# tenstack/batch-scheduler

Measured on AMD Instinct MI355X. Metric: pod x node fit evals/sec, higher is better.
Workload: dtype int64; 1 GPU; cfg3/tail: 10000 pods / 2000 groups / 5000 nodes, 5 int64 lanes (cpu, mem, eph, pods, gpu), seed 20260921; stages=prefilter+filter+tally+ready, parallelism=single GPU

## Files before the change

### batch-scheduler_amd/csrc/bs_fast.hpp

```cpp
#pragma once

#include "bs_kernels.hpp"
#include "bs_filter_t.hpp"

#ifdef BS_NT_TABLES
#define BS_TBL_STORE(p, v) __builtin_nontemporal_store((v), (p))
#else
#define BS_TBL_STORE(p, v) (*(p) = (v))
#endif
namespace bs {

template <bool INL = false>
__device__ __forceinline__ void arm_tally(const GroupsDev& gr, const BatchDev& b, const BatchParams& prm, uint32_t i, uint32_t nthreads);

__device__ __forceinline__ const uint8_t* range_glocal(const BatchDev& b) { return reinterpret_cast<const uint8_t*>(b.pod_ranges); }
__device__ __forceinline__ const uint32_t* range_start(const BatchDev& b, uint32_t G) { return b.pod_ranges + (G + 3u) / 4u; }
__device__ __forceinline__ const uint32_t* range_lfirst(const BatchDev& b, uint32_t G, uint32_t pod_blocks) { return range_start(b, G) + pod_blocks + 1u; }
__device__ __forceinline__ bool range_local_on(const BatchDev& b, const BatchParams& prm) {
  return b.pod_ranges && prm.do_tally && prm.do_ready && !prm.filter_deny;
}

#if BS_EMIT_MAIN
__global__ void k_pods_prep(unsigned long long* tables, uint32_t ntab, uint32_t* gstat, uint32_t ngstat, uint32_t* kcount, uint32_t* gcount, uint32_t G) {
  const uint32_t t = blockIdx.x * blockDim.x + threadIdx.x, nt = gridDim.x * blockDim.x;
// ... 201 lines not shown
    }
  }
  {
    const uint32_t grp = k >> 6;
    const bool grp_valid = (chunk * kTblChunk + (threadIdx.x & ~63u)) < nd.m;
    constexpr int64_t kSafe = (int64_t)1 << 62;
#pragma unroll
    for (uint32_t j = 0; j < BS_MAX_LANES; ++j) {
      if (j < L) {
        const int64_t x = (int64_t)incl[j];
        const long long mx = wave_max_i64_lane63(valid ? x : INT64_MIN);
        const bool risky = __ballot(valid && (x >= kSafe || x <= -kSafe)) != 0ull;
        if (lane_id() == 63 && grp_valid) b.gmax[(size_t)grp * LP + j] = risky ? INT64_MAX : mx;
      }
    }
  }
#pragma unroll
  for (uint32_t s = 0; s < BS_MAX_SCALARS; ++s) {
    if (s < S) {
      const unsigned long long mk = __ballot(valid && (pres & (1u << s)));
      if (mk && lane_id() == 0) atomicMin(&s_kp[s], chunk * kTblChunk + (uint32_t)(threadIdx.x & ~63u) + (uint32_t)(__ffsll((long long)mk) - 1));
    }
  }
  __syncthreads();
  if (threadIdx.x < 16) b.chunk_kp[(size_t)chunk * 16 + threadIdx.x] = threadIdx.x < BS_MAX_SCALARS ? s_kp[threadIdx.x] : BS_INF;
}

struct LeaderPre { Res mr; bool have_mr; int64_t min_member, status_scheduled, matched; };
template <bool PUB, typename T>
__device__ __forceinline__ void st_pub(T* p, T v) {
  if constexpr (PUB) __hip_atomic_store(p, v, __ATOMIC_RELAXED, __HIP_MEMORY_SCOPE_AGENT);
  else *p = v;
}
#ifndef BS_HOME_WT
#define BS_HOME_WT 0
#endif
template <typename T>
__device__ __forceinline__ void st_home(T* p, T v) {
#if BS_HOME_WT
  __hip_atomic_store(p, v, __ATOMIC_RELAXED, __HIP_MEMORY_SCOPE_SYSTEM);
#else
  *p = v;
#endif
}
__device__ __forceinline__ uint32_t ld_agent(const uint32_t* p) { return __hip_atomic_load(p, __ATOMIC_RELAXED, __HIP_MEMORY_SCOPE_AGENT); }
__device__ __forceinline__ unsigned long long ld_agent64(const void* p) {
  return __hip_atomic_load(reinterpret_cast<const unsigned long long*>(p), __ATOMIC_RELAXED, __HIP_MEMORY_SCOPE_AGENT);
}
template <int TS>
__device__ __forceinline__ void leader_pre_load(const GroupsDev& gr, int32_t leader, Shape<TS> sh, LeaderPre& o) {
  const uint32_t l = leader >= 0 ? (uint32_t)leader : 0u;
#pragma unroll
  for (uint32_t j = 0; j < BS_MAX_LANES; ++j) o.mr.v[j] = j < sh.L() ? gr.minres[(size_t)j * gr.g + l] : 0;
  o.mr.present = gr.mrpres[l];
  o.have_mr = (gr.flags[l] & BS_GROUP_HAS_MINRES) != 0;
  o.min_member = (int64_t)gr.min_member[l];
  o.status_scheduled = (int64_t)gr.status_scheduled[l];
  o.matched = (int64_t)gr.matched[l];
}
template <int TS>
__device__ __forceinline__ void pre_allocated_from(const LeaderPre& lp, Shape<TS> sh, uint32_t gate, Res& out) {
  res_zero(out, sh);
  const int64_t mm = lp.min_member;
  const int64_t not_finished = lp.matched != 0 ? mm - lp.matched : mm - lp.status_scheduled;
  if (not_finished > 0 && lp.have_mr) {
    Res times;
#pragma unroll
    for (uint32_t j = 0; j < BS_MAX_LANES; ++j)
      if (j < sh.L()) times.v[j] = wmul(lp.mr.v[j], not_finished);
    times.present = lp.mr.present;
    res_add(out, times, sh, gate);
  }
  if (out.v[BS_LANE_PODS] == 0) out.v[BS_LANE_PODS] = mm + 1;
}
template <int TS>
__device__ __forceinline__ uint32_t filter_slot_values(const Res& cur_in, const LeaderPre& lp, Shape<TS> sh, uint32_t gate, int64_t (&R)[4], int64_t (&M)[4]) {
  Res ms, cur = cur_in;
  res_zero(ms, sh);
  res_add(ms, lp.mr, sh, gate);
  res_add(cur, ms, sh, gate);
  uint32_t ff = 0;
#pragma unroll
  for (uint32_t s = 0; s < BS_MAX_SCALARS; ++s) {
    if (s < sh.S()) {
      if ((cur.present & (1u << s)) && cur.v[4 + s] != 0) ff |= 1u;
      if ((ms.present & (1u << s)) && ms.v[4 + s] != 0) ff |= 2u;
    }
  }
#pragma unroll
  for (int j = 0; j < 4; ++j) { R[j] = cur.v[j]; M[j] = ms.v[j]; }
  return ff;
}
template <int TS, bool PUB = false>
__device__ __forceinline__ void filter_slot_from(const BatchDev& b, const BatchParams& prm, const Res& cur_in, const LeaderPre& lp, Shape<TS> sh, uint32_t gate,
                                                 uint32_t slot, bool zero_feas = true) {
  if (!lp.have_mr) return;
  int64_t R[4], M[4];
  const uint32_t ff = filter_slot_values(cur_in, lp, sh, gate, R, M);
  if (zero_feas) st_pub<PUB>(&b.fu_feas[slot], 0u);
  int64_t* dst2 = b.uparams + (size_t)slot * 8;
#pragma unroll
  for (int j = 0; j < 4; ++j) { st_pub<PUB>(&dst2[j], R[j]); st_pub<PUB>(&dst2[4 + j], M[j]); }
  st_pub<PUB>(&b.uflags[slot], ff | ((uint32_t)BS_FL_EVALUATED << 8) | (prm.stamp << 16));
}
template <int TS>
__device__ __forceinline__ uint32_t class_scan_query(const Res& cur, const LeaderPre& lp0, Shape<TS> sh, uint32_t gate, Res& q) {
  pre_allocated_from(lp0, sh, gate, q);
  res_add(q, cur, sh, gate);
  uint32_t absok = 0;
#pragma unroll
  for (uint32_t s2 = 0; s2 < BS_MAX_SCALARS; ++s2) {
    if (s2 < sh.S()) {
      const bool pres = q.present & (1u << s2);
      if (!pres || q.v[4 + s2] == 0) absok |= 1u << s2;
      if (!pres) q.v[4 + s2] = INT64_MIN;
    }
  }
  return q.present | (absok << 16);
}

template <int TS, bool PUB = false, bool SLOTS = true, bool INL = false>
__device__ __forceinline__ void fast_query_thread(const PodsDev& pods, const GroupsDev& gr, const BatchDev& b, const BatchParams& prm, uint32_t i,
                                                  uint32_t nthreads, uint32_t end = BS_INF, uint32_t t = BS_INF) {
  const Shape<TS> sh(prm.S);
  const bool valid = i < pods.p && i < end;
  const uint32_t gate = prm.eph_gate;
  const uint32_t ii = valid ? i : 0u;
  const int32_t leader0 = b.leader_epoch[0];
  const uint8_t panic0 = b.panic_epoch[0];
  const uint32_t K = prm.run_filter ? (prm.k_host ? prm.k_host : *b.kclass) : 0u;
  const int32_t gi = pods.p ? pods.group[ii] : BS_POD_NOT_GROUPED;
  const uint8_t pfl = pods.p ? pods.flags[ii] : (uint8_t)0;
  const uint64_t own = pods.p ? pods.owner[ii] : 0ull;
  const uint32_t pc = pods.p ? b.pclass[ii] : 0u;
  const uint32_t pp = pods.p ? b.ppair[ii] : BS_INF;
  Res cur;
  if (pods.p) pod_require(pods, ii, sh, gate, cur); else res_zero(cur, sh);
  arm_tally<INL>(gr, b, prm, t == BS_INF ? i : t, nthreads);
  if (i < 8 && prm.collect_stats) b.stats[i] = 0;
  const bool grouped = valid && gi >= 0 && (uint32_t)gi < gr.g;
  const uint32_t g = grouped ? (uint32_t)gi : 0u;
  const uint8_t gfl = gr.g ? gr.flags[g] : (uint8_t)0;
  const uint64_t occ0 = gr.g ? gr.occupied[g] : 0ull;
  const uint32_t fo = gr.g ? b.first_owner_s[g] : BS_INF;
  const uint32_t anchor = grouped ? b.first_pod_s[g] : i;
  LeaderPre lp0{}, lp1{};
  const bool two = prm.run_filter && prm.sop_leader0 >= 0 && prm.sop_leader0 != leader0;
  if (gr.g) {
    leader_pre_load(gr, leader0, sh, lp0);
    if (two) leader_pre_load(gr, prm.sop_leader0, sh, lp1); else lp1 = lp0;
  }
  const bool need_fo = grouped && occ0 == 0 && fo != BS_INF && i > fo;
  const uint64_t occ_fo = need_fo ? pods.owner[fo] : 0ull;
  const uint32_t owner_rank = valid ? owner_rank_of(b, prm, anchor, pods.p) : 0u;

  uint8_t code = BS_PF_PASS_NOT_GROUPED, st = 0;
  bool has_q = false;
  Res q;
  res_zero(q, sh);
  if (valid) {
    if (owner_rank == prm.rank) st |= ST_OWNED;
    if (gi == BS_POD_NOT_GROUPED) code = BS_PF_PASS_NOT_GROUPED;
    else if (pfl & BS_POD_LAST_PERMITTED) code = BS_PF_PASS_LAST_PERMITTED;
    else if (!grouped) code = BS_PF_ERR_PG_NOT_FOUND;
    else if ((gfl & BS_GROUP_DENIED) || fd_denied(b, (uint32_t)gi, i)) code = BS_PF_ERR_DENIED;
    else {
      st |= ST_ELIG;
      bool occ_err = false;
      if (occ0 != 0) occ_err = (own == 0) || (own != occ0);
      else if (need_fo) occ_err = (own == 0) || (own != occ_fo);
      if (occ_err) code = BS_PF_ERR_OCCUPIED;
      else if (panic0) code = BS_PF_PANIC_DIV0;
      else {
        st |= ST_REACH6;
        if (leader0 < 0) code = BS_PF_PASS_NO_MAX;
        else if (leader0 == gi) code = BS_PF_PASS_IS_MAX;
        else {
          pre_allocated_from(lp0, sh, gate, q);
          res_add(q, cur, sh, gate);
          code = BS_PF_PASS_RESERVE_FITS;
          has_q = (st & ST_OWNED) != 0;
        }
      }
    }
    if (has_q) st |= ST_QUERY;
    b.tcode[i] = code;
    b.stage[i] = st;
  }
  BS_STAMP(1, 1);
  {
    __shared__ uint32_t s_reach;
    if (threadIdx.x == 0) s_reach = BS_INF;
    __syncthreads();
    const unsigned long long rb = __ballot(valid && (st & ST_REACH6));
    if (rb && lane_id() == __ffsll((long long)rb) - 1) atomicMin(&s_reach, i);
    __syncthreads();
    if (threadIdx.x == 0) st_pub<INL>(&b.first_reach64[blockIdx.x], ((unsigned long long)prm.seq_inv << 32) | s_reach);
  }
  BS_STAMP(1, 2);
  const uint32_t qslot = has_q ? pc : 0u;
  bool fill = SLOTS && wave_elect_by_key(qslot, has_q);
  bool w1 = false, w2 = false;
  if (SLOTS && prm.run_filter) {
    const bool may = valid && (st & ST_OWNED) && BS_PF_IS_PASS(code) && grouped;
    w1 = wave_elect_by_key(pc, may && leader0 >= 0 && leader0 != gi);
    w2 = wave_elect_by_key(pc, may && prm.sop_leader0 >= 0 && prm.sop_leader0 != gi);
  }
  if constexpr (PUB) {
    uint32_t o1 = 0, o2 = 0, o3 = 0;
    if (w1) o1 = __hip_atomic_exchange(&b.uclaim[pc], prm.stamp, __ATOMIC_RELAXED, __HIP_MEMORY_SCOPE_AGENT);
    if (w2) o2 = __hip_atomic_exchange(&b.uclaim[pc + K], prm.stamp, __ATOMIC_RELAXED, __HIP_MEMORY_SCOPE_AGENT);
    if (fill) o3 = __hip_atomic_exchange(&b.qstamp_s[qslot], prm.stamp, __ATOMIC_RELAXED, __HIP_MEMORY_SCOPE_AGENT);
    if (w1 && o1 == prm.stamp) w1 = false;
    if (w2 && o2 == prm.stamp) w2 = false;
    if (fill && o3 == prm.stamp) fill = false;
  }
  if (w1) filter_slot_from<TS, PUB>(b, prm, cur, lp0, sh, gate, pc);
  if (w2) filter_slot_from<TS, PUB>(b, prm, cur, lp1, sh, gate, pc + K);
  BS_STAMP(1, 3);
  if (has_q) {
    b.qpos[i] = qslot;
    atomicMin(&b.pair_firstq[pp], ((unsigned long long)prm.seq_inv << 32) | i);
  }
  if (fill) {
    uint32_t absok = 0;
#pragma unroll
    for (uint32_t s = 0; s < BS_MAX_SCALARS; ++s) {
      if (s < sh.S()) {
        const bool pres = q.present & (1u << s);
        if (!pres || q.v[4 + s] == 0) absok |= 1u << s;
        if (!pres) q.v[4 + s] = INT64_MIN;
      }
    }
    const uint32_t slot = qslot;
    int64_t* dst = b.qreq_s + (size_t)slot * prm.LP;
#pragma unroll
    for (uint32_t j = 0; j < BS_MAX_LANES; ++j)
      if (j < prm.LP) st_pub<PUB>(&dst[j], j < sh.L() ? q.v[j] : (int64_t)INT64_MIN);
    st_pub<PUB>(&b.qflags_s[slot], q.present | (absok << 16));
    st_pub<PUB>(&b.qtab_s[slot], (int32_t)0);
    st_pub<PUB>(&b.first_row[slot], BS_INF);
    st_pub<PUB>(&b.qstamp_s[slot], prm.stamp);
  }
  if (prm.collect_stats) {
    const unsigned long long hq = __ballot(has_q);
    if (lane_id() == 0 && hq) atomicAdd((unsigned long long*)&b.stats[2], (unsigned long long)__popcll(hq));
  }
}

template <int TS>
__device__ __forceinline__ void node_words_block(const GroupsDev& gr, const NodesDev& nd, const BatchDev& b, const BatchParams& prm, uint32_t blk) {
  const Shape<TS> sh(prm.S);
  const uint32_t gate = prm.eph_gate;
  const uint32_t n = blk * kTblChunk + threadIdx.x, w = nodew_wave_word(blk, threadIdx.x), stride = b.nodew_stride;
  const bool stores = nodew_wave_stores(nd.n, w) && lane_id() == 0;
  const int32_t leaders[2] = {b.leader_epoch[0], prm.sop_leader0};
  int64_t l[4] = {INT64_MIN, INT64_MIN, INT64_MIN, INT64_MIN};
  uint8_t fl = 0xFF;
  if (n < nd.n) {
#pragma unroll
    for (int j = 0; j < 4; ++j) l[j] = nd.left4[(size_t)j * nd.stride + n];
    fl = nd.flags[n];
  }
  const unsigned long long ok = __ballot(fl != 0xFF && !(fl & (BS_NODE_NIL | BS_NODE_NO_NODE)));
  if (stores) {
    b.nodew[nodew_pair(stride, 2, w)] = ok;
    b.nodew[nodew_pair(stride, 2, w) + 1] = ~0ull;
  }
#pragma unroll
  for (int s = 0; s < 2; ++s) {
    LeaderPre lp{};
    const bool have = gr.g != 0 && leaders[s] >= 0;
    if (have) leader_pre_load(gr, leaders[s], sh, lp);
    Res ms;
    res_zero(ms, sh);
    if (have && lp.have_mr) res_add(ms, lp.mr, sh, gate);
    uint32_t ff = (have && lp.have_mr) ? 1u : 0u;
#pragma unroll
    for (uint32_t q = 0; q < BS_MAX_SCALARS; ++q)
      if (q < sh.S() && (ms.present & (1u << q)) && ms.v[4 + q] != 0) ff |= 2u;
    const unsigned long long holds = __ballot(l[0] >= ms.v[0] && l[1] >= ms.v[1] && l[2] >= ms.v[2] && l[3] >= ms.v[3]);
    if (stores) {
      b.nodew[nodew_pair(stride, s, w)] = ok;
      b.nodew[nodew_pair(stride, s, w) + 1] = ~holds;
    }
    if (blk == 0 && threadIdx.x == 0) {
#pragma unroll
      for (int j = 0; j < 4; ++j) b.nodew[nodew_ref_lane(stride, s, j)] = (uint64_t)ms.v[j];
      b.nodew[nodew_ref_flags(stride, s)] = ff;
    }
  }
}

template <int TS>
__global__ __launch_bounds__(kTblChunk) void k_fast_query_tables(PodsDev pods, GroupsDev gr, NodesDev nd, BatchDev b, BatchDev bt, BatchParams prm,
                                                                 const TableDesc* forced, uint32_t nchunks, uint32_t query_blocks) {
  BS_STAMP(1, 0);
  if (blockIdx.x < query_blocks) fast_query_thread<TS>(pods, gr, b, prm, blockIdx.x * kTblChunk + threadIdx.x, query_blocks * kTblChunk);
  else if (blockIdx.x < query_blocks + nchunks) tables_local_fast<TS>(nd, bt, prm, forced, blockIdx.x - query_blocks);
  else node_words_block<TS>(gr, nd, b, prm, blockIdx.x - query_blocks - nchunks);
  BS_STAMP(1, 7);
}

template <int NL>
__device__ __forceinline__ unsigned long long rows_cover(unsigned long long m, const int64_t (&a)[BS_MAX_LANES], const int64_t (&r)[BS_MAX_LANES]) {
  asm volatile("s_mov_b64 exec, %[m]\n\tv_cmpx_ge_i64 vcc, %[a0], %[r0]\n\tv_cmpx_ge_i64 vcc, %[a1], %[r1]\n\tv_cmpx_ge_i64 vcc, %[a2], %[r2]\n\t"
               "v_cmpx_ge_i64 vcc, %[a3], %[r3]\n\ts_mov_b64 %[m], exec\n\ts_mov_b64 exec, -1"
               : [m] "+s"(m)
               : [a0] "v"(a[0]), [r0] "v"(r[0]), [a1] "v"(a[1]), [r1] "v"(r[1]), [a2] "v"(a[2]), [r2] "v"(r[2]), [a3] "v"(a[3]), [r3] "v"(r[3])
               : "vcc");
#pragma unroll
  for (int j = 4; j < NL; ++j)
    asm volatile("s_mov_b64 exec, %[m]\n\tv_cmpx_ge_i64 vcc, %[a], %[r]\n\ts_mov_b64 %[m], exec\n\ts_mov_b64 exec, -1" : [m] "+s"(m) : [a] "v"(a[j]), [r] "v"(r[j]) : "vcc");
  return m;
}
#ifndef BS_SCAN_BALLOT
#define BS_SCAN_BALLOT 1
#endif
constexpr uint32_t kSpinBound = 1u << 18;
__device__ __forceinline__ void test_chaos_delay() {
#ifdef BS_TEST_CHAOS
  uint32_t h = (blockIdx.x + 1u) * 2654435761u ^ (uint32_t)wall_clock64() * 40503u;
  h ^= h >> 15; h *= 2246822519u; h ^= h >> 13;
  for (uint32_t s = 0; s < (h & 15u); ++s) __builtin_amdgcn_s_sleep(127);
#endif
}
constexpr uint32_t kStepSlotsMax = 256;
__device__ __forceinline__ bool step_wait(const uint32_t* word, uint32_t base, uint32_t need, int32_t* h_err) {
  uint32_t spins = 0;
  while ((uint32_t)(ld_agent(word) - base) < need) {
    __builtin_amdgcn_s_sleep(1);
    if (++spins > kSpinBound) { if (h_err) __hip_atomic_store(h_err, 1, __ATOMIC_RELAXED, __HIP_MEMORY_SCOPE_SYSTEM); return false; }
  }
  return true;
}
constexpr uint32_t kScanRecChunks = 64;
constexpr uint32_t kFeasRecGroups = 32;
#ifndef BS_GATHER_DIRECT
#define BS_GATHER_DIRECT 8
#endif
constexpr uint32_t kGatherDirectBlocks = BS_GATHER_DIRECT;
constexpr uint32_t kRecStride = 32;
constexpr uint32_t kTkSlots = 32, kTkTab = 48, kTkP1 = 64, kTkDone = 64 + 16 * 16, kTkWays = 16, kTkWords = 64 + 2 * 16 * 16;
__device__ __forceinline__ void spread_add(uint32_t* words, uint32_t who) {
  (void)__hip_atomic_fetch_add(&words[16u * (who % kTkWays)], 1u, __ATOMIC_RELAXED, __HIP_MEMORY_SCOPE_AGENT);
}
__device__ __forceinline__ bool spread_wait(const uint32_t* words, uint32_t base, uint32_t need, int32_t* h_err) {
  uint32_t spins = 0;
  for (;;) {
    uint32_t v = lane_id() < (int)kTkWays ? ld_agent(&words[16u * (uint32_t)lane_id()]) : 0u;
#pragma unroll
    for (int o = 1; o < (int)kTkWays; o <<= 1) v += (uint32_t)__shfl_xor((int)v, o);
    v = (uint32_t)__builtin_amdgcn_readfirstlane((int)v);
    if ((uint32_t)(v - base) >= need) return true;
    __builtin_amdgcn_s_sleep(4);
    if (++spins > kSpinBound) { if (h_err && lane_id() == 0) __hip_atomic_store(h_err, 1, __ATOMIC_RELAXED, __HIP_MEMORY_SCOPE_SYSTEM); return false; }
  }
}
template <int TS, bool REGS = false>
__device__ __forceinline__ void table_scan_block(const NodesDev& nd, const BatchDev& b, const BatchParams& prm, const TableDesc* forced, uint32_t chunk, uint32_t nchunks,
                                                 uint32_t share, uint32_t nshares, uint32_t pod_blocks, uint32_t tk_pods0, uint32_t tk_tab0, const GroupsDev& gr,
                                                 const int64_t* ckeys, const uint32_t* cpres, uint32_t kcap, bool direct = false, uint32_t forced_cls = 0) {
  __shared__ unsigned long long s_wtot[BS_MAX_LANES][4];
  __shared__ uint32_t s_kp[BS_MAX_SCALARS];
  __shared__ unsigned long long s_off[BS_MAX_LANES];
  __shared__ uint32_t s_kpg[BS_MAX_SCALARS];
  __shared__ int64_t s_req[kStepSlotsMax][BS_MAX_LANES];
  __shared__ uint32_t s_qf[kStepSlotsMax];
  __shared__ uint32_t s_first[kStepSlotsMax];
  BS_STAMP(2, 0);
  const Shape<TS> sh(prm.S);
  const uint32_t L = sh.L(), S = sh.S(), LP = prm.LP;
  const uint32_t k = chunk * kTblChunk + threadIdx.x;
  const bool in_range = REGS ? k < nd.n : k < nd.m;
  const uint32_t n = REGS ? (in_range ? k : 0u) : (in_range ? nd.kmap[k] : 0u);
  const TableDesc d = REGS ? TableDesc{forced_cls, 0.7f} : *forced;
  const uint32_t fw = nd.fit[(size_t)d.cls * nd.fit_words + (n >> 5)];
  const uint8_t fl = nd.flags[n];
  const bool valid = in_range && (!REGS || !(fl & BS_NODE_SKIP_MASK));
  const uint32_t ap = nd.apres[n], rp = nd.rpres[n];
  int64_t al[BS_MAX_LANES], rq[BS_MAX_LANES];
#pragma unroll
  for (uint32_t j = 0; j < BS_MAX_LANES; ++j) {
    if (j < L) {
      al[j] = nd.alloc[(size_t)j * nd.stride + n];
      rq[j] = nd.req[(size_t)j * nd.stride + n];
    }
  }
  const uint32_t K = prm.k_host ? prm.k_host : *b.kclass;
  const uint32_t per = (K + nshares - 1u) / nshares, s_lo = share * per, s_hi = min(K, s_lo + per);
  Res raw;
  int32_t leader0 = -1;
  uint8_t panic0 = 0;
  LeaderPre lp0{};
  if constexpr (REGS) {
    const uint32_t cc = s_lo + threadIdx.x < s_hi ? s_lo + threadIdx.x : 0u;
#pragma unroll
    for (uint32_t j = 0; j < BS_MAX_LANES; ++j)
      if (j < L) raw.v[j] = ckeys[(size_t)j * kcap + cc];
    raw.present = cpres[cc];
    leader0 = b.leader_epoch[0];
    panic0 = b.panic_epoch[0];
    if (gr.g) leader_pre_load(gr, leader0, sh, lp0);
  }
  const bool fit = valid && ((fw >> (n & 31u)) & 1u) && !(fl & BS_NODE_TAINT_ERR);
  const uint32_t pres = fit ? (ap & rp) : 0u;
  if (threadIdx.x < BS_MAX_SCALARS) s_kp[threadIdx.x] = BS_INF;
  for (uint32_t t = threadIdx.x; t < kStepSlotsMax; t += kTblChunk) s_first[t] = BS_INF;
  unsigned long long incl[BS_MAX_LANES];
  const int w = wave_id();
#pragma unroll
  for (uint32_t j = 0; j < BS_MAX_LANES; ++j) {
    incl[j] = 0;
    if (j < L) {
      const bool live = fit && (j < 4 || (pres & (1u << (j - 4)))) && !(j == BS_LANE_EPH && !prm.eph_gate);
      const unsigned long long left = live ? (unsigned long long)wsub(scale_f32(al[j], d.pct), rq[j]) : 0ull;
      incl[j] = wave_incl_scan_add_u64(left);
      if (lane_id() == 63) s_wtot[j][w] = incl[j];
    }
  }
  __syncthreads();
#pragma unroll
  for (uint32_t s2 = 0; s2 < BS_MAX_SCALARS; ++s2) {
    if (s2 < S) {
      const unsigned long long mk = __ballot(valid && (pres & (1u << s2)));
      if (mk && lane_id() == 0) atomicMin(&s_kp[s2], chunk * kTblChunk + (uint32_t)(threadIdx.x & ~63u) + (uint32_t)(__ffsll((long long)mk) - 1));
    }
  }
#pragma unroll
  for (uint32_t j = 0; j < BS_MAX_LANES; ++j) {
    if (j < L) {
      unsigned long long off = 0, tot = 0;
#pragma unroll
      for (int i = 0; i < 4; ++i) {
        const unsigned long long x = s_wtot[j][i];
        if (i < w) off += x;
        tot += x;
      }
      incl[j] += off;
      if (threadIdx.x == 0 && share == 0) {
        if constexpr (REGS) {
          const unsigned long long tag = (unsigned long long)prm.seq_inv << 32;
          st_pub<true>(&b.chunk_rec[(size_t)chunk * kRecStride + 2u * j], tag | (uint32_t)tot);
          st_pub<true>(&b.chunk_rec[(size_t)chunk * kRecStride + 2u * j + 1u], tag | (uint32_t)(tot >> 32));
        } else {
          st_pub<true>(&b.chunk_tot[(size_t)chunk * 16 + j], tot);
        }
      }
    }
  }
  __syncthreads();
  __shared__ uint32_t s_ok;
  if constexpr (REGS) {
    if (share == 0 && threadIdx.x < S) st_pub<true>(&b.chunk_rec[(size_t)chunk * kRecStride + 16u + threadIdx.x], ((unsigned long long)prm.seq_inv << 32) | s_kp[threadIdx.x]);
    BS_STAMP(2, 1);
  } else {
    if (share == 0 && threadIdx.x < 16) st_pub<true>(&b.chunk_kp[(size_t)chunk * 16 + threadIdx.x], threadIdx.x < BS_MAX_SCALARS ? s_kp[threadIdx.x] : BS_INF);
    asm volatile("s_waitcnt vmcnt(0)" ::: "memory");
    __syncthreads();
    BS_STAMP(2, 1);
    if (threadIdx.x == 0 && share == 0) (void)__hip_atomic_fetch_add(&b.ticket[kTkTab], 1u, __ATOMIC_RELAXED, __HIP_MEMORY_SCOPE_AGENT);
  }
  if constexpr (REGS) {
    const uint32_t t = s_lo + threadIdx.x;
    if (t < s_hi) {
      uint32_t qf = 0x80000000u;
      Res q;
      res_zero(q, sh);
      if (leader0 >= 0 && !panic0) {
        Res cur;
        res_zero(cur, sh);
        res_add(cur, raw, sh, prm.eph_gate);
        qf = class_scan_query(cur, lp0, sh, prm.eph_gate, q);
      }
      s_qf[threadIdx.x] = qf;
#pragma unroll
      for (uint32_t j = 0; j < BS_MAX_LANES; ++j)
        if (j < L) s_req[threadIdx.x][j] = q.v[j];
    }
  }
  if constexpr (!REGS) {
    if (threadIdx.x == 0) s_ok = (step_wait(&b.ticket[kTkTab], tk_tab0, nchunks, b.h_err) && step_wait(&b.ticket[kTkSlots], tk_pods0, pod_blocks, b.h_err)) ? 1u : 0u;
    __syncthreads();
    BS_STAMP(2, 2);
    if (!s_ok) return;
  }
  {
    const uint32_t ch = (uint32_t)lane_id();
    unsigned long long cv[BS_MAX_LANES];
    uint32_t ckp[BS_MAX_SCALARS];
    if constexpr (REGS) {
      if (w == 0) {
        const uint32_t tagw = prm.seq_inv;
        const unsigned long long* rec = b.chunk_rec + (size_t)(ch < nchunks ? ch : 0u) * kRecStride;
        bool ok = false;
        for (uint32_t spins = 0;; ++spins) {
          unsigned long long lo[BS_MAX_LANES], hi[BS_MAX_LANES], kw[BS_MAX_SCALARS];
#pragma unroll
          for (uint32_t j = 0; j < BS_MAX_LANES; ++j)
            if (j < L) { lo[j] = ld_agent64(&rec[2u * j]); hi[j] = ld_agent64(&rec[2u * j + 1u]); }
#pragma unroll
          for (uint32_t s2 = 0; s2 < BS_MAX_SCALARS; ++s2)
            if (s2 < S) kw[s2] = ld_agent64(&rec[16u + s2]);
          bool mine_ok = true;
#pragma unroll
          for (uint32_t j = 0; j < BS_MAX_LANES; ++j) {
            cv[j] = 0ull;
            if (j < L) {
              mine_ok = mine_ok && (uint32_t)(lo[j] >> 32) == tagw && (uint32_t)(hi[j] >> 32) == tagw;
              cv[j] = (hi[j] << 32) | (uint32_t)lo[j];
            }
          }
#pragma unroll
          for (uint32_t s2 = 0; s2 < BS_MAX_SCALARS; ++s2) {
            ckp[s2] = BS_INF;
            if (s2 < S) { mine_ok = mine_ok && (uint32_t)(kw[s2] >> 32) == tagw; ckp[s2] = (uint32_t)kw[s2]; }
          }
          if (__ballot(!(mine_ok || ch >= nchunks)) == 0ull) { ok = true; break; }
          if (spins > kSpinBound) { if (b.h_err && ch == 0) __hip_atomic_store(b.h_err, 1, __ATOMIC_RELAXED, __HIP_MEMORY_SCOPE_SYSTEM); break; }
          __builtin_amdgcn_s_sleep(2);
        }
        if (ch >= nchunks) {
#pragma unroll
          for (uint32_t j = 0; j < BS_MAX_LANES; ++j) cv[j] = 0ull;
#pragma unroll
          for (uint32_t s2 = 0; s2 < BS_MAX_SCALARS; ++s2) ckp[s2] = BS_INF;
        }
        if (ch == 0) s_ok = ok ? 1u : 0u;
      }
      BS_STAMP(2, 2);
    } else if (w == 0) {
#pragma unroll
      for (uint32_t j = 0; j < BS_MAX_LANES; ++j) cv[j] = (j < L && ch < nchunks) ? ld_agent64(&b.chunk_tot[(size_t)ch * 16 + j]) : 0ull;
#pragma unroll
      for (uint32_t s2 = 0; s2 < BS_MAX_SCALARS; ++s2) ckp[s2] = (s2 < S && ch < nchunks) ? ld_agent(&b.chunk_kp[(size_t)ch * 16 + s2]) : BS_INF;
    }
    const uint32_t t = s_lo + threadIdx.x;
    uint32_t stp = 0, qf = 0x80000000u;
    int32_t tab = -1;
    unsigned long long rv[BS_MAX_LANES];
    if (!REGS && t < s_hi) {
      stp = ld_agent(&b.qstamp_s[t]);
      tab = (int32_t)ld_agent(reinterpret_cast<const uint32_t*>(&b.qtab_s[t]));
      qf = ld_agent(&b.qflags_s[t]);
#pragma unroll
      for (uint32_t j = 0; j < BS_MAX_LANES; ++j) rv[j] = j < L ? ld_agent64(&b.qreq_s[(size_t)t * LP + j]) : 0ull;
    }
    if (w == 0) {
#pragma unroll
      for (uint32_t j = 0; j < BS_MAX_LANES; ++j) {
        if (j < L) {
          const unsigned long long incl_c = wave_incl_scan_add_u64(cv[j]);
          const unsigned long long mine = bcast64(incl_c - cv[j], (int)(chunk & 63u));
          if (ch == 0) s_off[j] = mine;
        }
      }
#pragma unroll
      for (uint32_t s2 = 0; s2 < BS_MAX_SCALARS; ++s2) {
        if (s2 < S) {
          const uint32_t mn = wave_min_u32(ckp[s2]);
          if (ch == 0) s_kpg[s2] = mn;
        }
      }
    }
    if (!REGS && t < s_hi) {
      if (stp != prm.stamp || tab != 0) qf = 0x80000000u;
      s_qf[threadIdx.x] = qf;
#pragma unroll
      for (uint32_t j = 0; j < BS_MAX_LANES; ++j)
        if (j < L) s_req[threadIdx.x][j] = (int64_t)rv[j];
    }
  }
  __syncthreads();
  if constexpr (REGS) {
    if (!s_ok) return;
  }
  int64_t fin[BS_MAX_LANES];
  uint32_t keyrow = 0;
#pragma unroll
  for (uint32_t j = 0; j < BS_MAX_LANES; ++j) {
    fin[j] = 0;
    if (j < L) fin[j] = (int64_t)(incl[j] + s_off[j]);
  }
#pragma unroll
  for (uint32_t s2 = 0; s2 < BS_MAX_SCALARS; ++s2)
    if (s2 < S && k >= s_kpg[s2]) keyrow |= 1u << s2;
  BS_STAMP(2, 3);
  const uint32_t nmine = s_hi > s_lo ? s_hi - s_lo : 0u;
  const uint32_t smask = S ? ((1u << S) - 1u) : 0u;
  const uint32_t row0 = chunk * kTblChunk + ((uint32_t)w << 6);
  for (uint32_t t0 = 0; t0 < nmine; t0 += 4u) {
    uint32_t qf[4];
    int64_t r[4][BS_MAX_LANES];
#pragma unroll
    for (uint32_t u = 0; u < 4; ++u) {
      const uint32_t t = min(t0 + u, nmine - 1u);
      qf[u] = t0 + u < nmine ? s_qf[t] : 0x80000000u;
#pragma unroll
      for (uint32_t j = 0; j < BS_MAX_LANES; ++j) r[u][j] = j < L ? s_req[t][j] : 0;
    }
#pragma unroll
    for (uint32_t u = 0; u < 4; ++u) {
      const uint32_t nab = ~(qf[u] >> 16) & smask;
      unsigned long long m = (qf[u] & 0x80000000u) ? 0ull : __ballot(valid && (nab & ~keyrow) == 0u);
      static_assert(TS >= 0 && TS <= 4, "k_fast_step_a is instantiated for 0..4 scalar lanes (run_fast: step_a_possible)");
#if BS_SCAN_BALLOT
#pragma unroll
      for (uint32_t j = 0; j < 4u + (uint32_t)TS; ++j) m &= __ballot(fin[j] >= r[u][j]);
#else
      m = rows_cover<4 + TS>(m, fin, r[u]);
#endif
      if (m && lane_id() == 0) atomicMin(&s_first[t0 + u], row0 + (uint32_t)(__ffsll((long long)m) - 1));
    }
  }
  __syncthreads();
  BS_STAMP(2, 4);
  if constexpr (REGS) {
    if (direct) {
      for (uint32_t t = threadIdx.x; t < nmine; t += kTblChunk)
        st_pub<true>(&b.scan_rec[(size_t)chunk * kStepSlotsMax + s_lo + t], ((unsigned long long)prm.seq_inv << 32) | s_first[t]);
    } else {
      for (uint32_t t = threadIdx.x; t < nmine; t += kTblChunk)
        if (s_first[t] != BS_INF) atomicMin(&b.first_row64[s_lo + t], ((unsigned long long)prm.seq_inv << 32) | s_first[t]);
    }
    BS_STAMP(2, 7);
    return;
  }
  for (uint32_t t = threadIdx.x; t < nmine; t += kTblChunk) {
    if (s_first[t] == BS_INF) continue;
    atomicMin(&b.first_row[s_lo + t], s_first[t]);
  }
  BS_STAMP(2, 7);
}

__device__ __forceinline__ void step_filter_split(uint32_t K, uint32_t W, uint32_t target_waves, uint32_t& tiles, uint32_t& bpw, uint32_t& nchunk) {
  tiles = (2u * K + 63u) / 64u;
  uint32_t nsplit = max(1u, target_waves / max(tiles, 1u));
  nsplit = min(nsplit, max((W + 1u) / 2u, 1u));
  bpw = max(2u, (((W + nsplit - 1u) / nsplit + 1u) / 2u) * 2u);
  nchunk = (W + bpw - 1u) / bpw;
  if ((nchunk + 3u) / 4u > kFeasRecGroups) {
    bpw = ((W + 4u * kFeasRecGroups - 1u) / (4u * kFeasRecGroups) + 1u) / 2u * 2u;
    nchunk = (W + bpw - 1u) / bpw;
  }
}
template <int TS>
__device__ __forceinline__ void step_filter_block(const GroupsDev& gr, const NodesDev& nd, const BatchDev& b, const BatchParams& prm, const int64_t* ckeys,
                                                  const uint32_t* cpres, uint32_t kcap, uint32_t target_waves, uint32_t ustride, uint32_t bx, uint32_t nblocks,
                                                  bool direct, uint32_t tk_slots0, uint32_t slot_producers) {
  __shared__ uint32_t s_cnt[4][64];
  BS_STAMP_AT(4, 0, bx);
  const Shape<TS> sh(prm.S);
  const uint32_t gate = prm.eph_gate, K = prm.k_host ? prm.k_host : (uint32_t)__builtin_amdgcn_readfirstlane((int)*b.kclass), U = 2u * K;
  const uint32_t W = (nd.n + 63u) / 64u;
  if (!U || !W) return;
  uint32_t tiles, bpw, nchunk;
  step_filter_split(K, W, target_waves, tiles, bpw, nchunk);
  const uint32_t groups = (nchunk + 3u) / 4u;
  const int32_t leader0 = b.leader_epoch[0];
  LeaderPre lp0{}, lp1{};
  const bool two = prm.sop_leader0 >= 0 && prm.sop_leader0 != leader0;
  if (gr.g) {
    leader_pre_load(gr, leader0, sh, lp0);
    if (two) leader_pre_load(gr, prm.sop_leader0, sh, lp1); else lp1 = lp0;
  }
  bool waited = false;
  for (uint32_t bi = bx; bi < tiles * groups; bi += nblocks) {
    const uint32_t tile = bi % tiles, group = bi / tiles, chunk = group * 4u + (uint32_t)wave_id();
    const uint32_t src = tile * 64u + (uint32_t)lane_id();
    const bool second = src >= K;
    const uint32_t c = src < U ? (second ? src - K : src) : 0u;
    uint32_t cnt = 0;
    if (chunk < nchunk) {
      Res raw;
#pragma unroll
      for (uint32_t j = 0; j < BS_MAX_LANES; ++j)
        if (j < sh.L()) raw.v[j] = ckeys[(size_t)j * kcap + c];
      raw.present = cpres[c];
      Res cur;
      res_zero(cur, sh);
      res_add(cur, raw, sh, gate);
      LeaderPre lp = lp0;
      if (second) lp = lp1;
      const bool on = src < U && (second ? prm.sop_leader0 >= 0 : leader0 >= 0) && lp.have_mr;
      int64_t R[4], M[4];
      const uint32_t ff = filter_slot_values(cur, lp, sh, gate, R, M);
      filter_item<2, 4, true, true>(nd, b, U, ustride, tile, chunk * bpw, min(W, chunk * bpw + bpw), 0u,
                                    on ? (ff | ((uint32_t)BS_FL_EVALUATED << 8)) : ((uint32_t)BS_FL_NOT_RUN << 8), R, M, &cnt);
    }
    s_cnt[wave_id()][lane_id()] = cnt;
    BS_STAMP_AT(4, 1, bx);
    if (direct && b.h_rows) asm volatile("s_waitcnt vmcnt(0)" ::: "memory");
    __syncthreads();
    BS_STAMP_AT(4, 2, bx);
    if (wave_id() == 0 && src < U) {
      const uint32_t sum = s_cnt[0][lane_id()] + s_cnt[1][lane_id()] + s_cnt[2][lane_id()] + s_cnt[3][lane_id()];
      if (direct) {
        st_pub<true>(&b.feas_rec[(size_t)group * (2u * kStepSlotsMax) + src], ((unsigned long long)prm.seq_inv << 32) | sum);
      } else {
        if (!waited) { (void)step_wait(&b.ticket[kTkSlots], tk_slots0, slot_producers, b.h_err); waited = true; }
        if (sum) atomicAdd(&b.fu_feas[src], sum);
      }
    }
    __syncthreads();
  }
  BS_STAMP_AT(4, 7, bx);
}

template <int TS>
__device__ __forceinline__ void class_slots_block(const GroupsDev& gr, const BatchDev& b, const BatchParams& prm, const int64_t* ckeys, const uint32_t* cpres,
                                                  uint32_t kcap, uint32_t blk, bool zero_feas) {
  const Shape<TS> sh(prm.S);
#ifdef BS_TEST_OLD_ZERO
  zero_feas = true;
#endif
  const uint32_t gate = prm.eph_gate, K = prm.k_host ? prm.k_host : *b.kclass;
  const uint32_t c = blk * kTblChunk + threadIdx.x;
  Res raw;
  const uint32_t cc = c < K ? c : 0u;
#pragma unroll
  for (uint32_t j = 0; j < BS_MAX_LANES; ++j)
    if (j < sh.L()) raw.v[j] = ckeys[(size_t)j * kcap + cc];
  raw.present = cpres[cc];
  const int32_t leader0 = b.leader_epoch[0];
  const uint8_t panic0 = b.panic_epoch[0];
  LeaderPre lp0{}, lp1{};
  const bool two = prm.run_filter && prm.sop_leader0 >= 0 && prm.sop_leader0 != leader0;
  if (gr.g) {
    leader_pre_load(gr, leader0, sh, lp0);
    if (two) leader_pre_load(gr, prm.sop_leader0, sh, lp1); else lp1 = lp0;
  }
  if (c < K) {
    Res cur;
    res_zero(cur, sh);
    res_add(cur, raw, sh, gate);
    if (leader0 >= 0 && !panic0) {
      Res q;
      const uint32_t qfw = class_scan_query(cur, lp0, sh, gate, q);
      int64_t* dst = b.qreq_s + (size_t)c * prm.LP;
#pragma unroll
      for (uint32_t j = 0; j < BS_MAX_LANES; ++j)
        if (j < prm.LP) st_pub<true>(&dst[j], j < sh.L() ? q.v[j] : (int64_t)INT64_MIN);
      st_pub<true>(&b.qflags_s[c], qfw);
      st_pub<true>(&b.qtab_s[c], (int32_t)0);
      st_pub<true>(&b.first_row[c], BS_INF);
      st_pub<true>(&b.qstamp_s[c], prm.stamp);
    }
    if (prm.run_filter) {
      if (leader0 >= 0) filter_slot_from<TS, true>(b, prm, cur, lp0, sh, gate, c, zero_feas);
      if (prm.sop_leader0 >= 0) filter_slot_from<TS, true>(b, prm, cur, lp1, sh, gate, c + K, zero_feas);
    }
  }
  BS_STAMP(1, 4);
  asm volatile("s_waitcnt vmcnt(0)" ::: "memory");
  __syncthreads();
  BS_STAMP(1, 5);
  if (threadIdx.x == 0) (void)__hip_atomic_fetch_add(&b.ticket[kTkSlots], 1u, __ATOMIC_RELAXED, __HIP_MEMORY_SCOPE_AGENT);
}


template <bool INL>
__device__ __forceinline__ void arm_tally(const GroupsDev& gr, const BatchDev& b, const BatchParams& prm, uint32_t i, uint32_t nthreads) {
  if (i == 0) __hip_atomic_store(&b.ticket[1], 0u, __ATOMIC_RELAXED, __HIP_MEMORY_SCOPE_AGENT);
  for (uint32_t g = i; g < gr.g; g += nthreads) {
    if (INL && range_local_on(b, prm) && range_glocal(b)[g]) continue;
    st_pub<INL>(&b.admit[g], 0u);
    if (prm.do_ready) {
      st_pub<INL>(&b.admit64[g], 0ull);
      if (b.gcount[g] == 0u) {
        const uint8_t rd = gr.matched[g] >= (uint32_t)(gr.min_member[g] - gr.status_scheduled[g]) ? 1 : 0;
        b.ready[g] = rd;
        if (prm.host_tag) { st_home(&b.h_admit[g], 0u); st_home(&b.h_ready[g], rd); }
      }
    }
  }
}

template <bool WT = false>
__device__ __forceinline__ void final_tail(const BatchDev& b, const BatchParams& prm, uint32_t nblocks) {
  __shared__ uint32_t s_last;
  if (!prm.host_tag) return;
  if constexpr (WT && BS_HOME_WT) asm volatile("s_waitcnt vmcnt(0)" ::: "memory");
  else __builtin_amdgcn_fence(__ATOMIC_RELEASE, "");
  __syncthreads();
  if (threadIdx.x == 0) s_last = __hip_atomic_fetch_add(&b.ticket[0], 1u, __ATOMIC_RELAXED, __HIP_MEMORY_SCOPE_AGENT) == nblocks - 1 ? 1u : 0u;
  __syncthreads();
  if (!s_last) return;
  if (threadIdx.x == 0) {
    __hip_atomic_store(&b.ticket[0], 0u, __ATOMIC_RELAXED, __HIP_MEMORY_SCOPE_AGENT);
    if constexpr (WT && BS_HOME_WT) __hip_atomic_store(b.h_tag, prm.host_tag, __ATOMIC_RELAXED, __HIP_MEMORY_SCOPE_SYSTEM);
    else __hip_atomic_store(b.h_tag, prm.host_tag, __ATOMIC_RELEASE, __HIP_MEMORY_SCOPE_SYSTEM);
  }
}

__device__ __forceinline__ void tally_quorum_atomic(const BatchDev& b, const BatchParams& prm, bool grouped, uint32_t g, bool admit, uint32_t want, uint32_t ma,
                                                    uint32_t need) {
  unsigned long long mine = 0;
  bool asked = false;
  unsigned long long todo = __ballot(grouped);
  const unsigned long long adm = __ballot(grouped && admit);
  for (int round = 0; todo && round < kElectRounds; ++round) {
    const int leader = __ffsll((long long)todo) - 1;
    const uint32_t k0 = (uint32_t)__builtin_amdgcn_readlane((int)g, leader);
    const unsigned long long same = __ballot(grouped && g == k0) & todo;
    if (lane_id() == leader) {
      mine = ((unsigned long long)__popcll(same) << 32) | (unsigned long long)__popcll(same & adm);
      asked = true;
    }
    todo &= ~same;
  }
  if (todo & (1ull << lane_id())) {
    mine = (1ull << 32) | (admit ? 1ull : 0ull);
    asked = true;
  }
  unsigned long long got = 0;
  if (asked) got = __hip_atomic_fetch_add(&b.admit64[g], mine, __ATOMIC_RELAXED, __HIP_MEMORY_SCOPE_AGENT);
  if (asked) {
    const unsigned long long tot = got + mine;
    if ((uint32_t)(tot >> 32) == want) {
      const uint32_t ad = (uint32_t)tot;
      const uint8_t rd = (ma + ad) >= need ? 1 : 0;
      b.admit[g] = ad;
      b.ready[g] = rd;
      if (prm.host_tag) { st_home(&b.h_admit[g], ad); st_home(&b.h_ready[g], rd); }
    }
  }
}
template <bool WT = false>
__device__ __forceinline__ void tally_tail(const GroupsDev& gr, const BatchDev& b, const BatchParams& prm, bool grouped, uint32_t g, bool admit,
                                           uint32_t nblocks) {
  if (prm.do_tally && prm.do_ready) {
    uint32_t want = 0, ma = 0, mm = 0, sc = 0;
    if (grouped) { want = b.gcount[g]; ma = gr.matched[g]; mm = gr.min_member[g]; sc = gr.status_scheduled[g]; }
    tally_quorum_atomic(b, prm, grouped, g, admit, want, ma, (uint32_t)(mm - sc));
  } else if (prm.do_tally) {
    wave_aggregated_add(b.admit, g, grouped && admit);
  }
  final_tail<WT>(b, prm, nblocks);
}

constexpr uint32_t kLocalTag = 0x80000000u;
template <bool WT = false>
__device__ __forceinline__ void tally_tail_whole(const GroupsDev& gr, const BatchDev& b, const BatchParams& prm, bool grouped, uint32_t g, bool admit,
                                                 uint32_t nblocks, uint32_t gwant, uint32_t ma, uint32_t need, uint32_t* s_adm) {
  if (prm.do_tally && prm.do_ready) {
    const bool local = grouped && (gwant & kLocalTag);
    const uint32_t lslot = gwant & 0xFFu;
    if (local && admit) atomicAdd(&s_adm[lslot], 1u);
    __syncthreads();
    if (local && lslot == threadIdx.x) {
      const uint32_t ad = s_adm[lslot];
      const uint8_t rd = (ma + ad) >= need ? 1 : 0;
      b.admit[g] = ad;
      b.ready[g] = rd;
      if (prm.host_tag) { st_home(&b.h_admit[g], ad); st_home(&b.h_ready[g], rd); }
    }
    tally_quorum_atomic(b, prm, grouped && !local, g, admit, gwant, ma, need);
  } else if (prm.do_tally) {
    wave_aggregated_add(b.admit, g, grouped && admit);
  }
  final_tail<WT>(b, prm, nblocks);
}


template <bool INL = false>
__device__ __forceinline__ void fast_final_block(const PodsDev& pods, const GroupsDev& gr, const NodesDev& nd, const BatchDev& b, const BatchParams& prm,
                                                 uint32_t query_blocks, uint32_t bx, uint32_t nblocks, uint32_t producers, uint32_t tk_p1 = 0, uint32_t aux = 0,
                                                 uint32_t tk_done = 0, uint32_t hint_blocks = 0, uint32_t p0 = BS_INF, uint32_t p1 = BS_INF) {
  __shared__ uint32_t s_first_reach;
  __shared__ uint32_t s_rowk[INL ? kStepSlotsMax : 1u], s_feask[INL ? 2u * kStepSlotsMax : 1u], s_ladm[INL ? 256u : 1u], s_gw[INL ? 3u : 1u][INL ? 256u : 1u];
  BS_STAMP(3, 0);
  if constexpr (INL) {
    s_ladm[threadIdx.x] = 0u;
    if (threadIdx.x < 64) (void)spread_wait(&b.ticket[kTkP1], tk_p1, query_blocks, b.h_err);
    __syncthreads();
  }
  const uint32_t dx = bx * 256u + threadIdx.x;
  const uint32_t i = p0 == BS_INF ? dx : p0 + threadIdx.x;
  const bool valid = i < pods.p && (p0 == BS_INF || i < p1);
  uint8_t code0 = 0, st0 = 0;
  int32_t gi0 = BS_POD_NOT_GROUPED;
  uint32_t qpos0 = 0, pclass0 = 0, pair0 = BS_INF;
  uint32_t lfirst = BS_INF;
  if (valid) { code0 = b.tcode[i]; st0 = b.stage[i]; gi0 = pods.group[i]; qpos0 = b.qpos[i]; pclass0 = b.pclass[i]; pair0 = b.ppair[i]; }
  if (INL && valid && range_local_on(b, prm)) lfirst = range_lfirst(b, gr.g, query_blocks)[i];
  const uint32_t K = prm.k_host ? prm.k_host : *b.kclass;
  const int32_t leader_now = b.leader_epoch[0];
  if (threadIdx.x < 64) {
    uint32_t found = BS_INF;
    for (uint32_t b0 = 0; b0 < query_blocks && found == BS_INF; b0 += 64u) {
      const uint32_t bk = b0 + threadIdx.x;
      uint32_t v = BS_INF;
      if (bk < query_blocks) {
        const unsigned long long w = INL ? ld_agent64(&b.first_reach64[bk]) : b.first_reach64[bk];
        if ((uint32_t)(w >> 32) == prm.seq_inv) v = (uint32_t)w;
      }
      const unsigned long long any = __ballot(v != BS_INF);
      if (any) found = (uint32_t)__shfl((int)v, __ffsll((long long)any) - 1);
    }
    if (threadIdx.x == 0) s_first_reach = found;
  }
  const bool owned = valid && (st0 & ST_OWNED);
  const bool walk = owned && (st0 & ST_ELIG);
  const bool grouped = valid && gi0 >= 0 && (uint32_t)gi0 < gr.g;
  uint32_t row_q = BS_INF, row_c = BS_INF, feas0 = 0, feas1 = 0;
  unsigned long long head = ~0ull, own_fq = ~0ull, own_next = ~0ull;
  if (walk) {
    head = b.pair_head[gi0];
    if (pair0 != BS_INF) { own_fq = INL ? ld_agent64(&b.pair_firstq[pair0]) : b.pair_firstq[pair0]; own_next = b.pair_next[pair0]; }
  }
  if constexpr (INL) {
    if (prm.do_tally && prm.do_ready) {
      uint32_t gwant = 0, gma = 0, gneed = 0;
      if (grouped) {
        gma = gr.matched[gi0];
        gneed = (uint32_t)(gr.min_member[gi0] - gr.status_scheduled[gi0]);
// ... 419 lines not shown
```

Before: 3771 billion evals/s.

## Broadcast per-pod requests via readlane in register table scan

In the REGS path, pod request vectors are now stored in shared memory in a transposed lane-major layout. Each wavefront loads up to 64 pods' requests and flags in one coalesced read per lane, then broadcasts each pod to the wave with readlane instead of every lane re-reading shared memory. Node validity and scalar-key checks are precomputed once as ballot masks rather than re-evaluated per pod. This trades LDS broadcast traffic for many scalar readlane operations and a serial per-pod loop, which may or may not be cheaper.

Result: slower. 3560 billion evals/s (-5.6%).

```diff
diff --git a/batch-scheduler_amd/csrc/bs_fast.hpp b/batch-scheduler_amd/csrc/bs_fast.hpp
--- a/batch-scheduler_amd/csrc/bs_fast.hpp
+++ b/batch-scheduler_amd/csrc/bs_fast.hpp
@@ -593,6 +593,7 @@
   __shared__ int64_t s_req[kStepSlotsMax][BS_MAX_LANES];
   __shared__ uint32_t s_qf[kStepSlotsMax];
   __shared__ uint32_t s_first[kStepSlotsMax];
+  [[maybe_unused]] int64_t (*const s_req_t)[kStepSlotsMax] = reinterpret_cast<int64_t (*)[kStepSlotsMax]>(&s_req[0][0]);
   BS_STAMP(2, 0);
   const Shape<TS> sh(prm.S);
   const uint32_t L = sh.L(), S = sh.S(), LP = prm.LP;
@@ -701,7 +702,7 @@
       s_qf[threadIdx.x] = qf;
 #pragma unroll
       for (uint32_t j = 0; j < BS_MAX_LANES; ++j)
-        if (j < L) s_req[threadIdx.x][j] = q.v[j];
+        if (j < L) s_req_t[j][threadIdx.x] = q.v[j];
     }
   }
   if constexpr (!REGS) {
@@ -814,7 +815,39 @@
   const uint32_t nmine = s_hi > s_lo ? s_hi - s_lo : 0u;
   const uint32_t smask = S ? ((1u << S) - 1u) : 0u;
   const uint32_t row0 = chunk * kTblChunk + ((uint32_t)w << 6);
-  for (uint32_t t0 = 0; t0 < nmine; t0 += 4u) {
+  if constexpr (REGS) {
+    const unsigned long long mvalid = __ballot(valid);
+    unsigned long long mkey[TS > 0 ? TS : 1];
+#pragma unroll
+    for (uint32_t s2 = 0; s2 < (uint32_t)TS; ++s2) mkey[s2] = __ballot((keyrow >> s2) & 1u);
+    for (uint32_t p0 = 0; p0 < nmine; p0 += 64u) {
+      const uint32_t cnt = min(64u, nmine - p0);
+      const uint32_t tl = min(p0 + (uint32_t)lane_id(), nmine - 1u);
+      const uint32_t qfl = s_qf[tl];
+      int64_t rl[4 + TS];
+#pragma unroll
+      for (uint32_t j = 0; j < 4u + (uint32_t)TS; ++j) rl[j] = s_req_t[j][tl];
+      uint32_t res = BS_INF;
+      for (uint32_t u = 0; u < cnt; ++u) {
+        const uint32_t qf = (uint32_t)__builtin_amdgcn_readlane((int)qfl, (int)u);
+        const uint32_t nab = ~(qf >> 16) & smask;
+        unsigned long long m = (qf & 0x80000000u) ? 0ull : mvalid;
+#pragma unroll
+        for (uint32_t s2 = 0; s2 < (uint32_t)TS; ++s2)
+          if (nab & (1u << s2)) m &= mkey[s2];
+#pragma unroll
+        for (uint32_t j = 0; j < 4u + (uint32_t)TS; ++j) {
+          const uint32_t lo = (uint32_t)__builtin_amdgcn_readlane((int)(uint32_t)(uint64_t)rl[j], (int)u);
+          const uint32_t hi = (uint32_t)__builtin_amdgcn_readlane((int)(uint32_t)((uint64_t)rl[j] >> 32), (int)u);
+          m &= __ballot(fin[j] >= (int64_t)(((uint64_t)hi << 32) | lo));
+        }
+        const uint32_t first = m ? row0 + (uint32_t)(__ffsll((long long)m) - 1) : BS_INF;
+        res = (uint32_t)lane_id() == u ? first : res;
+      }
+      if ((uint32_t)lane_id() < cnt) atomicMin(&s_first[p0 + (uint32_t)lane_id()], res);
+    }
+  }
+  for (uint32_t t0 = 0; !REGS && t0 < nmine; t0 += 4u) {
     uint32_t qf[4];
     int64_t r[4][BS_MAX_LANES];
 #pragma unroll
```

## Transpose request staging and broadcast per-slot requirements via readlane in scan

Applied to the files above, without the earlier changes.

Stores the staged request vectors in a lane-major shared layout so each lane loads one slot's requirements with conflict-free accesses. The scan loop then processes 64 slots per outer iteration, broadcasting each slot's requirement through scalar readlane instead of re-reading shared memory for every slot. Scalar-key masks are precomputed once as ballots, and each slot's first-fit lane is gathered with s_ff1 and writelane. It issues one atomicMin per lane instead of one per slot. The inline-asm cmpx variant is removed, and the code now relies on raw intrinsics and asm whose correctness depends on uniform control flow.

Measured after the change: 3745 billion evals/s before, 3802 billion evals/s after (median of 6 runs). 1.02x the previous value.

```diff
diff --git a/batch-scheduler_amd/csrc/bs_fast.hpp b/batch-scheduler_amd/csrc/bs_fast.hpp
--- a/batch-scheduler_amd/csrc/bs_fast.hpp
+++ b/batch-scheduler_amd/csrc/bs_fast.hpp
@@ -527,21 +527,7 @@
   BS_STAMP(1, 7);
 }
 
-template <int NL>
-__device__ __forceinline__ unsigned long long rows_cover(unsigned long long m, const int64_t (&a)[BS_MAX_LANES], const int64_t (&r)[BS_MAX_LANES]) {
-  asm volatile("s_mov_b64 exec, %[m]\n\tv_cmpx_ge_i64 vcc, %[a0], %[r0]\n\tv_cmpx_ge_i64 vcc, %[a1], %[r1]\n\tv_cmpx_ge_i64 vcc, %[a2], %[r2]\n\t"
-               "v_cmpx_ge_i64 vcc, %[a3], %[r3]\n\ts_mov_b64 %[m], exec\n\ts_mov_b64 exec, -1"
-               : [m] "+s"(m)
-               : [a0] "v"(a[0]), [r0] "v"(r[0]), [a1] "v"(a[1]), [r1] "v"(r[1]), [a2] "v"(a[2]), [r2] "v"(r[2]), [a3] "v"(a[3]), [r3] "v"(r[3])
-               : "vcc");
-#pragma unroll
-  for (int j = 4; j < NL; ++j)
-    asm volatile("s_mov_b64 exec, %[m]\n\tv_cmpx_ge_i64 vcc, %[a], %[r]\n\ts_mov_b64 %[m], exec\n\ts_mov_b64 exec, -1" : [m] "+s"(m) : [a] "v"(a[j]), [r] "v"(r[j]) : "vcc");
-  return m;
-}
-#ifndef BS_SCAN_BALLOT
-#define BS_SCAN_BALLOT 1
-#endif
+__device__ extern int bs_writelane(int val, int lane, int old) asm("llvm.amdgcn.writelane.i32");
 constexpr uint32_t kSpinBound = 1u << 18;
 __device__ __forceinline__ void test_chaos_delay() {
 #ifdef BS_TEST_CHAOS
@@ -590,7 +576,7 @@
   __shared__ uint32_t s_kp[BS_MAX_SCALARS];
   __shared__ unsigned long long s_off[BS_MAX_LANES];
   __shared__ uint32_t s_kpg[BS_MAX_SCALARS];
-  __shared__ int64_t s_req[kStepSlotsMax][BS_MAX_LANES];
+  __shared__ int64_t s_req[BS_MAX_LANES][kStepSlotsMax];
   __shared__ uint32_t s_qf[kStepSlotsMax];
   __shared__ uint32_t s_first[kStepSlotsMax];
   BS_STAMP(2, 0);
@@ -701,7 +687,7 @@
       s_qf[threadIdx.x] = qf;
 #pragma unroll
       for (uint32_t j = 0; j < BS_MAX_LANES; ++j)
-        if (j < L) s_req[threadIdx.x][j] = q.v[j];
+        if (j < L) s_req[j][threadIdx.x] = q.v[j];
     }
   }
   if constexpr (!REGS) {
@@ -793,7 +779,7 @@
       s_qf[threadIdx.x] = qf;
 #pragma unroll
       for (uint32_t j = 0; j < BS_MAX_LANES; ++j)
-        if (j < L) s_req[threadIdx.x][j] = (int64_t)rv[j];
+        if (j < L) s_req[j][threadIdx.x] = (int64_t)rv[j];
     }
   }
   __syncthreads();
@@ -813,30 +799,48 @@
   BS_STAMP(2, 3);
   const uint32_t nmine = s_hi > s_lo ? s_hi - s_lo : 0u;
   const uint32_t smask = S ? ((1u << S) - 1u) : 0u;
-  const uint32_t row0 = chunk * kTblChunk + ((uint32_t)w << 6);
-  for (uint32_t t0 = 0; t0 < nmine; t0 += 4u) {
-    uint32_t qf[4];
-    int64_t r[4][BS_MAX_LANES];
-#pragma unroll
-    for (uint32_t u = 0; u < 4; ++u) {
-      const uint32_t t = min(t0 + u, nmine - 1u);
-      qf[u] = t0 + u < nmine ? s_qf[t] : 0x80000000u;
-#pragma unroll
-      for (uint32_t j = 0; j < BS_MAX_LANES; ++j) r[u][j] = j < L ? s_req[t][j] : 0;
-    }
-#pragma unroll
-    for (uint32_t u = 0; u < 4; ++u) {
-      const uint32_t nab = ~(qf[u] >> 16) & smask;
-      unsigned long long m = (qf[u] & 0x80000000u) ? 0ull : __ballot(valid && (nab & ~keyrow) == 0u);
-      static_assert(TS >= 0 && TS <= 4, "k_fast_step_a is instantiated for 0..4 scalar lanes (run_fast: step_a_possible)");
-#if BS_SCAN_BALLOT
-#pragma unroll
-      for (uint32_t j = 0; j < 4u + (uint32_t)TS; ++j) m &= __ballot(fin[j] >= r[u][j]);
-#else
-      m = rows_cover<4 + TS>(m, fin, r[u]);
-#endif
-      if (m && lane_id() == 0) atomicMin(&s_first[t0 + u], row0 + (uint32_t)(__ffsll((long long)m) - 1));
-    }
+  const uint32_t row0 = chunk * kTblChunk + ((uint32_t)__builtin_amdgcn_readfirstlane(w) << 6);
+  static_assert(TS >= 0 && TS <= 4, "k_fast_step_a is instantiated for 0..4 scalar lanes (run_fast: step_a_possible)");
+  const unsigned long long vmask = __ballot(valid);
+  unsigned long long kmask[TS > 0 ? TS : 1];
+#pragma unroll
+  for (uint32_t s2 = 0; s2 < (uint32_t)TS; ++s2) kmask[s2] = __ballot(valid && ((keyrow >> s2) & 1u));
+  if constexpr (TS > 0) kmask[0] &= vmask;
+  const uint32_t ln = (uint32_t)lane_id();
+  const uint32_t nmine_u = (uint32_t)__builtin_amdgcn_readfirstlane((int)nmine);
+  for (uint32_t t0 = 0; t0 < nmine_u; t0 += 64u) {
+    const uint32_t cnt = min(nmine_u - t0, 64u);
+    const uint32_t tl = t0 + min(ln, cnt - 1u);
+    const uint32_t qfl = ln < cnt ? s_qf[tl] : 0x80000000u;
+    uint32_t rlo[4 + TS], rhi[4 + TS];
+#pragma unroll
+    for (uint32_t j = 0; j < 4u + (uint32_t)TS; ++j) {
+      const int64_t x = s_req[j][tl];
+      rlo[j] = (uint32_t)x;
+      rhi[j] = (uint32_t)((uint64_t)x >> 32);
+    }
+    uint32_t res = BS_INF;
+    for (uint32_t u0 = 0; u0 < cnt; u0 += 4u) {
+#pragma unroll
+      for (uint32_t v = 0; v < 4u; ++v) {
+        const uint32_t u = u0 + v;
+        const uint32_t nab = ~((uint32_t)__builtin_amdgcn_readlane((int)qfl, (int)u) >> 16) & smask;
+        unsigned long long m = vmask;
+        if constexpr (TS > 0) m = (nab & 1u) ? kmask[0] : vmask;
+#pragma unroll
+        for (uint32_t s2 = 1; s2 < (uint32_t)TS; ++s2) m &= ((nab >> s2) & 1u) ? kmask[s2] : ~0ull;
+#pragma unroll
+        for (uint32_t j = 0; j < 4u + (uint32_t)TS; ++j) {
+          const uint32_t lo = (uint32_t)__builtin_amdgcn_readlane((int)rlo[j], (int)u), hi = (uint32_t)__builtin_amdgcn_readlane((int)rhi[j], (int)u);
+          m &= __ballot(fin[j] >= (int64_t)(((uint64_t)hi << 32) | lo));
+        }
+        int ff;
+        asm("s_ff1_i32_b64 %0, %1" : "=s"(ff) : "s"(m));
+        res = (uint32_t)bs_writelane(ff, (int)u, (int)res);
+      }
+    }
+    const bool hit = !(qfl & 0x80000000u) && res != 0xFFFFFFFFu;
+    if (hit) atomicMin(&s_first[t0 + ln], row0 + res);
   }
   __syncthreads();
   BS_STAMP(2, 4);
```
